# chrismile/LineVis

Measured on AMD Instinct MI355X. Metric: Mrays/s, higher is better.
Workload: dtype f32

## Files before the change

include/linevis_hip.h:

```cpp
#ifndef LINEVIS_HIP_H
#define LINEVIS_HIP_H

#include <stdint.h>

#ifdef __cplusplus
extern "C" {
#endif

#define LV_OK 0
#define LV_E_INVALID (-1)
#define LV_E_HIP (-2)
#define LV_E_STATE (-3)
#define LV_E_CAPACITY (-4)

#define LV_RENDERING_MODE_PER_PIXEL_LINKED_LIST 2
#define LV_RENDERING_MODE_MLAB 3
#define LV_RENDERING_MODE_MBOIT 6
#define LV_RENDERING_MODE_VULKAN_RAY_TRACER 11

typedef struct lv_line_point {
    float linePosition[3];
    float lineAttribute;
    float lineTangent[3];
    float lineRotation;
// ... 5 lines not shown
    float vertexPosition[3];
    uint32_t vertexLinePointIndex;
    float vertexNormal[3];
    float phi;
} lv_tube_vertex;

typedef struct lv_stats {
    uint64_t rays_traced;
    uint64_t nodes_visited;
    uint64_t prims_tested;
    uint64_t hits_shaded;
    uint64_t fragments;
    uint64_t ao_hit_pixels;
    uint32_t max_depth_complexity;
    uint32_t bvh_depth;
    uint32_t num_segments;
    uint32_t num_nodes;
    float ms_accel_build;
    float ms_depth_range;
    float ms_ao;
    float ms_color;
    float ms_ppll_clear;
    float ms_ppll_gather;
    float ms_ppll_resolve;
    float ms_total;
    uint64_t device_bytes;
    float ms_kernel_avg[8];
    uint32_t kernel_launches[8];
    uint64_t ao_rays_traced;
    uint64_t ao_nodes_visited;
    uint64_t ao_prims_tested;
    uint64_t ao_phase_iterations[3];
    uint64_t ao_phase_lanes[3];
    uint32_t max_nodes_per_pixel;
    uint32_t num_tube_triangles;
    uint64_t ppll_pool_nodes;
    uint64_t ao_prim_hits;
    uint64_t ao_prim_may_axis;
    uint64_t ao_prim_may_both;
    float ms_tri_accel_build;
    float ms_tessellate;
    float ms_line_points;
    uint32_t num_tri_nodes;
    uint32_t tri_leaf_bytes;
    uint32_t mboit_degenerate_pixels;
} lv_stats;

#define LV_KERNEL_AO_PRIMARY 0
#define LV_KERNEL_AO_RAYS 1
#define LV_KERNEL_RENDER_RT 2
#define LV_KERNEL_PPLL_GATHER 3
#define LV_KERNEL_PPLL_RESOLVE 4
#define LV_KERNEL_DEPTH_RANGE 5
#define LV_KERNEL_PPLL_SHADE 6
#define LV_KERNEL_PPLL_RASTER 7

typedef struct lv_ctx lv_ctx;

lv_ctx* lv_create(int device_ordinal, int* err);
void lv_destroy(lv_ctx* ctx);
const char* lv_last_error(const lv_ctx* ctx);
const char* lv_version(void);

int lv_set_stream(lv_ctx* ctx, void* hip_stream);

int lv_set_lines(lv_ctx* ctx, const lv_line_point* points, uint32_t num_points,
// ... 116 lines not shown
```

linevis_amd/capi.py:

```python
import ctypes as C
import os

import numpy as np

_HERE = os.path.dirname(os.path.abspath(__file__))
LIB_PATH = os.environ.get("LV_LIB_PATH") or os.path.join(_HERE, "_lib", "liblinevis_hip.so")
HEADER_PATH = os.path.join(os.path.dirname(_HERE), "include", "linevis_hip.h")

LV_OK = 0
MODE_PPLL = 2
MODE_MLAB = 3
MODE_MBOIT = 6
MODE_RAY_TRACER = 11

LINE_POINT_DTYPE = np.dtype([("linePosition", "<f4", 3), ("lineAttribute", "<f4"),
                             ("lineTangent", "<f4", 3), ("lineRotation", "<f4"),
                             ("lineNormal", "<f4", 3), ("lineStartIndex", "<u4")])
assert LINE_POINT_DTYPE.itemsize == 48
TUBE_VERTEX_DTYPE = np.dtype([("vertexPosition", "<f4", 3), ("vertexLinePointIndex", "<u4"),
                              ("vertexNormal", "<f4", 3), ("phi", "<f4")])
assert TUBE_VERTEX_DTYPE.itemsize == 32


class Stats(C.Structure):
    _fields_ = [("rays_traced", C.c_uint64), ("nodes_visited", C.c_uint64), ("prims_tested", C.c_uint64),
                ("hits_shaded", C.c_uint64), ("fragments", C.c_uint64), ("ao_hit_pixels", C.c_uint64),
                ("max_depth_complexity", C.c_uint32), ("bvh_depth", C.c_uint32), ("num_segments", C.c_uint32),
                ("num_nodes", C.c_uint32),
                ("ms_accel_build", C.c_float), ("ms_depth_range", C.c_float), ("ms_ao", C.c_float),
                ("ms_color", C.c_float), ("ms_ppll_clear", C.c_float), ("ms_ppll_gather", C.c_float),
                ("ms_ppll_resolve", C.c_float), ("ms_total", C.c_float), ("device_bytes", C.c_uint64),
                ("ms_kernel_avg", C.c_float * 8), ("kernel_launches", C.c_uint32 * 8),
                ("ao_rays_traced", C.c_uint64), ("ao_nodes_visited", C.c_uint64), ("ao_prims_tested", C.c_uint64),
                ("ao_phase_iterations", C.c_uint64 * 3), ("ao_phase_lanes", C.c_uint64 * 3),
                ("max_nodes_per_pixel", C.c_uint32), ("num_tube_triangles", C.c_uint32),
                ("ppll_pool_nodes", C.c_uint64), ("ao_prim_hits", C.c_uint64), ("ao_prim_may_axis", C.c_uint64),
                ("ao_prim_may_both", C.c_uint64),
                ("ms_tri_accel_build", C.c_float), ("ms_tessellate", C.c_float), ("ms_line_points", C.c_float),
                ("num_tri_nodes", C.c_uint32), ("tri_leaf_bytes", C.c_uint32), ("mboit_degenerate_pixels", C.c_uint32)]

    def as_dict(self):
        d = {}
        for n, _ in self._fields_:
            v = getattr(self, n)
            d[n] = list(v) if hasattr(v, "__len__") else v
        return d


class StreamlineSettings(C.Structure):
    _fields_ = [("integration_method", C.c_uint32), ("integration_direction", C.c_uint32),
                ("time_step_scale", C.c_float), ("max_num_iterations", C.c_int32),
                ("termination_distance", C.c_float), ("minimum_length", C.c_float)]


class HelicitySeedingSettings(C.Structure):
    _fields_ = [("minimum_separation_distance", C.c_float), ("termination_check_type", C.c_uint32), ("loop_check_mode", C.c_uint32),
                ("termination_distance_self", C.c_float), ("seeding_subsampling_factor", C.c_int32)]

    def __init__(self, minimum_separation_distance=0.08, termination_check_type=1, loop_check_mode=1, termination_distance_self=1.0,
                 seeding_subsampling_factor=1):
        super().__init__(minimum_separation_distance, termination_check_type, loop_check_mode, termination_distance_self,
                         seeding_subsampling_factor)


INTEGRATION_METHODS = {"Explicit Euler": 0, "Implicit Euler": 1, "Heun": 2, "Midpoint": 3, "Runge-Kutta 4th Order": 4,
                       "Runge-Kutta-Fehlberg": 5}
INTEGRATION_DIRECTIONS = {"Forward": 0, "Backward": 1, "Forward & Backward": 2}
# ... 489 lines not shown
```

linevis_amd/csrc/lv_api.hip:

```cpp
#include <algorithm>
#include <cmath>
#include <cstdlib>
#include <cstring>

#include "lv_internal.h"

int lv_fail(lv_ctx* ctx, int code, const char* fmt, ...) {
    char buf[1024];
    va_list ap;
    va_start(ap, fmt);
    vsnprintf(buf, sizeof(buf), fmt, ap);
    va_end(ap);
    if (ctx) ctx->lastError = buf;
    return code;
}

int lv_buf_reserve(lv_ctx* ctx, LvDeviceBuffer& b, size_t bytes) {
    if (bytes == 0) bytes = 16;
    if (b.ptr && b.bytes >= bytes) return LV_OK;
    if (b.ptr) {
        LV_HIP(ctx, hipStreamSynchronize(ctx->stream));
        (void)hipFree(b.ptr);
        b.ptr = nullptr;
        b.bytes = 0;
// ... 876 lines not shown
    if (ctx->evFrameValid) {
        s.ms_total = s.ms_depth_range = s.ms_ao = 0.0f;
        s.ms_color = s.ms_ppll_clear = s.ms_ppll_gather = s.ms_ppll_resolve = 0.0f;
        if (ctx->evPhaseRecorded) {
            s.ms_total = ms(2, 3);
            s.ms_depth_range = ms(2, 5);
            s.ms_ao = ms(5, 7);
            if (ctx->lastMode == LV_RENDERING_MODE_VULKAN_RAY_TRACER) s.ms_color = ms(7, 3);
            else { s.ms_ppll_clear = ms(7, 11); s.ms_ppll_gather = ms(11, 13); s.ms_ppll_resolve = ms(13, 3); }
        }
        LvDevCountersHost hc;
        memset(&hc, 0, sizeof(hc));
        if (ctx->counters.ptr) {
            LV_HIP(ctx, hipMemcpy(&hc, ctx->counters.ptr, sizeof(hc), hipMemcpyDeviceToHost));
        }
        s.rays_traced = hc.rays;
        s.nodes_visited = hc.nodes;
        s.prims_tested = hc.prims;
        s.hits_shaded = hc.hits;
        s.fragments = hc.fragCounter;
        s.ao_hit_pixels = hc.aoCount;
        s.max_depth_complexity = hc.maxDepthComplexity;
        s.ao_rays_traced = hc.aoRays;
        s.ao_nodes_visited = hc.aoNodes;
        s.ao_prims_tested = hc.aoPrims;
        s.max_nodes_per_pixel = hc.maxNodesPerPixel;
        s.ao_prim_hits = hc.aoPrimHits;
        s.ao_prim_may_axis = hc.aoPrimMayAxis;
        s.ao_prim_may_both = hc.aoPrimMayBoth;
        s.mboit_degenerate_pixels = hc.mboitDegenerate;
        if (ctx->mboitStreamLast && hc.mboitOverflow)
            return lv_fail(ctx, LV_E_CAPACITY, "MBOIT (streamed): a pixel of the last frame is covered by more than 131071 kept fragments");
        for (int k = 0; k < 3; k++) { s.ao_phase_iterations[k] = hc.aoPhaseIters[k]; s.ao_phase_lanes[k] = hc.aoPhaseLanes[k]; }
    }
    for (int k = 0; k < 8; k++) { s.ms_kernel_avg[k] = 0.0f; s.kernel_launches[k] = 0; }
    for (int k = 0; k < lv_ctx::kNumKernels; k++) {
        const uint64_t n = ctx->kernelLaunches[k];
        const uint64_t m = n < uint64_t(lv_ctx::kRing) ? n : uint64_t(lv_ctx::kRing);
        double sum = 0.0;
        for (uint64_t i = 0; i < m; i++) {
            const uint64_t slot = (n - 1 - i) % lv_ctx::kRing;
            float t = 0.0f;
            if (hipEventElapsedTime(&t, ctx->evKernel[k][2 * slot], ctx->evKernel[k][2 * slot + 1]) == hipSuccess) sum += t;
        }
        s.ms_kernel_avg[k] = m ? float(sum / double(m)) : 0.0f;
        s.kernel_launches[k] = uint32_t(n);
    }
    uint64_t bytes = 0;
    for (const LvDeviceBuffer* b : lv_all_buffers(ctx)) bytes += b->bytes;
    s.device_bytes = bytes;
    *out = s;
    for (int r = 1; aggregate && r < lv_multi_num_ranks(ctx); r++) {
        lv_stats ps;
        const int rc = lv_get_stats_impl(lv_multi_rank(ctx, r), &ps, false);
        if (rc) return lv_fail(ctx, rc, "rank %d: %s", r, lv_multi_rank(ctx, r)->lastError.c_str());
        out->rays_traced += ps.rays_traced; out->nodes_visited += ps.nodes_visited; out->prims_tested += ps.prims_tested;
        out->hits_shaded += ps.hits_shaded; out->fragments += ps.fragments; out->ao_hit_pixels += ps.ao_hit_pixels;
        out->ao_rays_traced += ps.ao_rays_traced; out->ao_nodes_visited += ps.ao_nodes_visited; out->ao_prims_tested += ps.ao_prims_tested;
        out->ao_prim_hits += ps.ao_prim_hits; out->ao_prim_may_axis += ps.ao_prim_may_axis; out->ao_prim_may_both += ps.ao_prim_may_both;
        out->max_depth_complexity = ps.max_depth_complexity > out->max_depth_complexity ? ps.max_depth_complexity : out->max_depth_complexity;
        out->mboit_degenerate_pixels += ps.mboit_degenerate_pixels;
        out->device_bytes += ps.device_bytes;
    }
    (void)hipSetDevice(ctx->device);
    return LV_OK;
}
// ... 380 lines not shown
```

linevis_amd/csrc/lv_device.h:

```cpp
#pragma once

#include <hip/hip_runtime.h>
#include <stdint.h>

#include "../../include/linevis_hip.h"

#define LV_WAVE 64
#define LV_BLOCK 256
#define LV_LEAF_BIT 0x80000000u
#define LV_INVALID 0xFFFFFFFFu
#ifndef LV_STACK_LDS
#define LV_STACK_LDS 24
#endif
#define LV_STACK_SPILL 64
#ifndef LV_RT_MIN_WAVES
#define LV_RT_MIN_WAVES 4
#endif
#ifndef LV_GATHER_MIN_WAVES
#define LV_GATHER_MIN_WAVES 1
#endif
#ifndef LV_PRISM_MIN_WAVES
#define LV_PRISM_MIN_WAVES 3
#endif
#define LV_PPLL_DEAD 0xFFFFFFFFu
// ... 42 lines not shown
#endif
#ifndef LV_NODE_MIN_ACTIVE
#define LV_NODE_MIN_ACTIVE 24
#endif

#ifndef LV_HANDOVER_MAX_BUSY
#define LV_HANDOVER_MAX_BUSY 32
#endif
#ifndef LV_HANDOVER_MAX_BUSY_ALL
#define LV_HANDOVER_MAX_BUSY_ALL 48
#endif
#ifndef LV_HANDOVER_MAX_BUSY_DYN
#define LV_HANDOVER_MAX_BUSY_DYN 24
#endif

#ifndef LV_RESOLVE_LDS_MAX
#define LV_RESOLVE_LDS_MAX (64 * 1024)
#endif
#ifndef LV_RESOLVE_SLAB_GRID
#define LV_RESOLVE_SLAB_GRID 4096u
#endif
#ifndef LV_PPLL_CHUNK
#define LV_PPLL_CHUNK 256
#endif
#ifndef LV_PPLL_SLICES
#define LV_PPLL_SLICES 1
#endif

struct LvDevCounters {
    unsigned long long rays, nodes, prims, hits;
    unsigned long long aoRays, aoNodes, aoPrims;
    unsigned long long aoQueueHead;
    unsigned long long aoPhaseIters[3], aoPhaseLanes[3];
    uint32_t fragCounter;
    uint32_t aoCount;
    uint32_t maxDepthComplexity;
    uint32_t depthOrd[2];
    uint32_t maxNodesPerPixel;
    uint32_t fragAlloc;
    uint32_t prismDiscards;
    uint32_t mlatTraceCount;
    uint32_t ppllOverflowPixels;
    uint32_t prismListCount;
    unsigned long long aoPrimHits, aoPrimMayAxis, aoPrimMayBoth;
    uint32_t mlabLongPixels;
    uint32_t mlabSaturated;
    uint32_t mboitDegenerate;
    uint32_t mboitBoxOrd[6];
    uint32_t mboitOverflow;
};

struct f3 { float x, y, z; };
struct f4 { float x, y, z, w; };

__device__ __forceinline__ f3 mk3(float x, float y, float z) { f3 r; r.x = x; r.y = y; r.z = z; return r; }
__device__ __forceinline__ f3 operator+(f3 a, f3 b) { return mk3(a.x + b.x, a.y + b.y, a.z + b.z); }
__device__ __forceinline__ f3 operator-(f3 a, f3 b) { return mk3(a.x - b.x, a.y - b.y, a.z - b.z); }
__device__ __forceinline__ f3 operator*(f3 a, float s) { return mk3(a.x * s, a.y * s, a.z * s); }
__device__ __forceinline__ f3 operator*(float s, f3 a) { return mk3(s * a.x, s * a.y, s * a.z); }
__device__ __forceinline__ float dot3(f3 a, f3 b) { return (a.x * b.x + a.y * b.y) + a.z * b.z; }
__device__ __forceinline__ f3 cross3(f3 a, f3 b) {
    return mk3(a.y * b.z - b.y * a.z, a.z * b.x - b.z * a.x, a.x * b.y - b.x * a.y);
}
__device__ __forceinline__ float len3(f3 a) { return sqrtf(dot3(a, a)); }
__device__ __forceinline__ f3 norm3(f3 a) { float l = len3(a); return mk3(a.x / l, a.y / l, a.z / l); }
__device__ __forceinline__ float clampf(float x, float lo, float hi) { return fminf(fmaxf(x, lo), hi); }
// ... 260 lines not shown
```

linevis_amd/csrc/lv_render.hip:

```cpp
#include <algorithm>
#include <cmath>
#include <cstring>

#include "lv_internal.h"
#include "lv_trace.h"
#include "lv_tile.h"
#include "lv_mboit.h"

namespace {

#define LV_PRE_HITS 4u
template <bool STATS, int PRIM, int BANDS = LV_SHADE_PLAIN, bool PRE = false, int FAST = 0>
__global__ __launch_bounds__(LV_BLOCK, (STATS || PRIM == LV_PRIM_ELLIPTIC) ? 1 : LV_RT_MIN_WAVES) void k_render_rt(const LvUniforms U, const LvSceneDev S, const LvTiles T,
                                                        uint32_t* __restrict__ out, LvDevCounters* dc,
                                                        const uint2* __restrict__ firstHit = nullptr, const size_t firstHitStride = 0) {
    __shared__ unsigned s_stack[LV_STACK_LDS * LV_BLOCK];
    LV_COOP_SHARED(LV_BLOCK / LV_WAVE);
    LV_COOP_MEM(cm);
    LvPixel px;
    if (!lv_block_pixel(U, T, px)) return;
    const unsigned long long tg0 = lv_group_clock();
    const LvStackMem sm = lv_stack_mem(s_stack, S.stackOverflow);
    LvCounters cnt = {0, 0, 0, 0};
    const bool capped = U.useCappedTubes != 0 || U.lssGeometry != 0;
// ... 306 lines not shown

__global__ __launch_bounds__(LV_BLOCK) void k_ao_tile_scan(const uint32_t* __restrict__ tileCount, uint32_t numTiles,
                                                           uint32_t* __restrict__ tileBase, LvDevCounters* dc) {
    __shared__ uint32_t s_part[LV_BLOCK];
    const uint32_t per = (numTiles + LV_BLOCK - 1u) / LV_BLOCK;
    const uint32_t b = threadIdx.x * per, e = min(b + per, numTiles);
    uint32_t sum = 0;
    for (uint32_t i = b; i < e; i++) sum += tileCount[i];
    s_part[threadIdx.x] = sum;
    __syncthreads();
    if (threadIdx.x == 0) {
        uint32_t run = 0;
        for (uint32_t i = 0; i < LV_BLOCK; i++) { const uint32_t v = s_part[i]; s_part[i] = run; run += v; }
        tileBase[numTiles] = run;
        dc->aoCount = run;
        dc->aoQueueHead = 0ull;
    }
    __syncthreads();
    uint32_t run = s_part[threadIdx.x];
    for (uint32_t i = b; i < e; i++) { tileBase[i] = run; run += tileCount[i]; }
}

__device__ __forceinline__ size_t lv_ao_slot(const uint32_t* __restrict__ tileBase, uint32_t numTiles, const LvAoLayout& tileCapacity,
                                             uint32_t ordinal) {
    if (!tileBase) return ordinal;
    uint32_t lo = 0, hi = numTiles;
    while (hi - lo > 1u) {
        const uint32_t mid = (lo + hi) >> 1;
        if (tileBase[mid] <= ordinal) lo = mid; else hi = mid;
    }
    return lv_ao_group_base(tileCapacity, lo) + (ordinal - tileBase[lo]);
}

#ifndef LV_AO_KEY64
#define LV_AO_KEY64 0
#endif
#if LV_AO_KEY64
typedef unsigned long long lv_ao_key;
__device__ __forceinline__ lv_ao_key lv_ao_key_none(float aoRadius) { return ((unsigned long long)__float_as_uint(aoRadius) << 32) | 0xFFFFFFFFull; }
__device__ __forceinline__ lv_ao_key lv_ao_key_hit(float t, unsigned low) { return ((unsigned long long)__float_as_uint(t) << 32) | low; }
__device__ __forceinline__ float lv_ao_key_t(lv_ao_key key) { return __uint_as_float(unsigned(key >> 32)); }
#else
typedef unsigned lv_ao_key;
__device__ __forceinline__ lv_ao_key lv_ao_key_none(float aoRadius) { return __float_as_uint(aoRadius) + 1u; }
__device__ __forceinline__ lv_ao_key lv_ao_key_hit(float t, unsigned) { return __float_as_uint(t); }
__device__ __forceinline__ float lv_ao_key_t(lv_ao_key key) { return __uint_as_float(key); }
#endif

template <bool BAKE>
__device__ __forceinline__ void lv_ao_generate_ray(const LvUniforms& U, float4 g0, float4 g1, float4 g2, uint32_t smpIdx, uint32_t spp,
                                                   const uint2* __restrict__ lcgSkip, float2* gen) {
    const uint32_t pix = __float_as_uint(g1.w);
    const f3 pos = mk3(g0.x, g0.y, g0.z), T = mk3(g1.x, g1.y, g1.z), N = mk3(g2.x, g2.y, g2.z);
    const f3 B = cross3(N, T);
    uint32_t seed;
    if (BAKE) {
        const uint32_t sub = __float_as_uint(g2.w);
        const uint2 skip = lcgSkip[2u * (sub * spp + smpIdx)];
        seed = skip.x * lv_tea(pix , U.aoFrameNumber) + skip.y;
    } else {
        seed = lv_tea(pix, U.aoGlobalFrameNumber * spp + smpIdx);
    }
    const float xi0 = lv_rnd(seed), xi1 = lv_rnd(seed);
    float sn, cs;
    lv_sincos2pi(xi1, sn, cs);
    const float rs = sqrtf(1.0f - xi0 * xi0);
    const f3 smp = mk3(cs * rs, sn * rs, xi0);
    const f3 dirU = mk3((T.x * smp.x + B.x * smp.y) + N.x * smp.z, (T.y * smp.x + B.y * smp.y) + N.y * smp.z,
                        (T.z * smp.x + B.z * smp.y) + N.z * smp.z);
    const f3 d = norm3(dirU);
    const f3 o = BAKE ? pos : pos + d * g0.w;
    gen[0] = make_float2(o.x, o.y);
    gen[1] = make_float2(o.z, d.x);
    gen[2] = make_float2(d.y, d.z);
}

template <bool STATS, bool ANY_HIT, int PRIM, bool BAKE = false, bool LIT = false, bool PIXEL_GEN = false>
__global__ __launch_bounds__(LV_AO_BLOCK, LV_AO_MIN_WAVES) void k_ao_rays(const LvUniforms U, const LvSceneDev S,
                                                         const float4* __restrict__ gbuf, float* __restrict__ samples,
                                                         LvDevCounters* dc, const uint32_t* __restrict__ tileBase,
                                                         uint32_t numTiles, const LvAoLayout tileCapacity,
                                                         const uint2* __restrict__ lcgSkip = nullptr) {
    __shared__ unsigned s_stack[LV_AO_STACK_LDS * LV_AO_BLOCK];
    __shared__ float2 s_ray[3 * LV_AO_BLOCK];
    __shared__ float2 s_gen[3 * LV_AO_BLOCK];
    __shared__ unsigned s_queue[LV_AO_BLOCK / LV_WAVE][LV_AO_QCAP];
    __shared__ lv_ao_key s_key[LV_AO_BLOCK];
    __shared__ uint4 s_genState[PIXEL_GEN ? LV_AO_BLOCK / LV_WAVE : 1];

    const uint32_t spp = U.aoSamplesPerFrame;
    const unsigned long long total = (unsigned long long)(dc->aoCount) * spp;
    const unsigned chunk = total < (unsigned long long)gridDim.x * (LV_AO_BLOCK / LV_WAVE) * LV_AO_CHUNK * LV_AO_SMALL_CHUNKS ? LV_AO_CHUNK_SMALL
                                                                                                                             : LV_AO_CHUNK;
    const bool capped = U.useCappedTubes != 0;
    const float radius = U.radius;
    const unsigned lane = threadIdx.x & 63u, w = threadIdx.x >> 6;
    const unsigned long long below = (1ull << lane) - 1ull;
    float2* rayW = &s_ray[3 * LV_WAVE * w];
    float2* genW = &s_gen[3 * LV_WAVE * w];
    unsigned* queueW = s_queue[w];
    lv_ao_key* keyW = &s_key[LV_WAVE * w];
    uint4* genStateW = &s_genState[PIXEL_GEN ? w : 0];
    if (PIXEL_GEN && lane == 0) genStateW[0] = make_uint4(0u, 0u, 0u, 0u);
    const lv_ao_key keyInit = lv_ao_key_none(U.aoRadius);
    const float litSlack = PRIM == LV_PRIM_ELLIPTIC ? S.ellBandWidth * 1.001f : (PRIM == LV_PRIM_CAPSULE && LIT) ? radius * 1.001f : 0.0f;

    LvStackT<LV_AO_STACK_LDS, LV_AO_BLOCK> st;
    st.init(&s_stack[threadIdx.x], S.stackOverflow ? S.stackOverflow + (size_t(blockIdx.x) * LV_AO_BLOCK + threadIdx.x) : nullptr,
            gridDim.x * LV_AO_BLOCK);
    LvCounters cnt = {0, 0, 0, 0};
    unsigned long long phIt[3] = {0, 0, 0}, phLn[3] = {0, 0, 0};
    unsigned long long mayAxis = 0, mayBoth = 0, primHits = 0;

    unsigned long long chunkNext = 0, chunkEnd = 0, genBase = 0;
    unsigned genCount = 0, genPos = 0;
    unsigned head = 0, tail = 0;
    bool sourceDry = (S.numSegs == 0) || (total == 0);
    bool hasRay = false, enq = false;
    unsigned long long r = 0;
    f3 inv = mk3(0, 0, 0), oi = mk3(0, 0, 0);
    float best = 0.0f;
    unsigned cur = LV_INVALID, lastSeq = 0;
    unsigned owner = lane;
    constexpr unsigned TB = PRIM == LV_PRIM_TRIANGLE ? LV_AO_TEST_BATCH_TRI : LV_AO_TEST_BATCH;

    while (true) {
        {
            const bool isLeaf = tail - head < LV_WAVE && cur != LV_INVALID && (cur & LV_LEAF_BIT);
            const unsigned long long mL = __ballot(isLeaf);
            if (mL) {
                if (isLeaf) {
                    const unsigned idx = tail + unsigned(__popcll(mL & below));
                    queueW[idx % LV_AO_QCAP] = (owner << 26) | (cur & 0x03FFFFFFu);
                    lastSeq = idx;
                    enq = true;
                    cur = lv_pop_or_done(st);
                }
                tail += unsigned(__popcll(mL));
                if (tail - head < TB) continue;
            }
        }
        const bool canRefill = (genPos < genCount) || !sourceDry;
        const bool drain = !canRefill;
        if (!drain && hasRay && cur == LV_INVALID && (!enq || int(head - lastSeq) > 0)) {
            const lv_ao_key key = keyW[lane];
            float occ = 1.0f;
            if (key != keyInit) occ = U.aoUseDistance ? lv_ao_key_t(key) / U.aoRadius : 0.0f;
            samples[r] = occ;
            hasRay = false;
        }
        const unsigned long long mNode = __ballot(cur != LV_INVALID && !(cur & LV_LEAF_BIT));
        const unsigned long long mIdle = __ballot(!hasRay);
        const int nNode = __popcll(mNode), nIdle = __popcll(mIdle);
        const unsigned q = tail - head;

        if (q >= TB || (q > 0 && nNode == 0 && !(canRefill && nIdle > 0))) {
            const unsigned n = q < LV_WAVE ? q : LV_WAVE;
            __builtin_amdgcn_fence(__ATOMIC_ACQ_REL, "wavefront");
            if (STATS && lane == 0) { phIt[2]++; phLn[2] += n; }
            if (lane < n) {
                const unsigned e = queueW[(head + lane) % LV_AO_QCAP];
                const unsigned owner = e >> 26, leaf = e & 0x03FFFFFFu;
                const float2 r0 = rayW[3 * owner], r1 = rayW[3 * owner + 1], r2 = rayW[3 * owner + 2];
                if (STATS) cnt.prims += PRIM == LV_PRIM_TRIANGLE ? S.triLeafSize : 1u;
                float t; unsigned low;
                if (lv_leaf_test<PRIM, LIT ? 1 : 0>(S, leaf, mk3(r0.x, r0.y, r1.x), mk3(r1.y, r2.x, r2.y), radius, capped, t, low, 0.0f,
                                                    U.aoRadius)) {
                    if (t >= 0.0f && t <= U.aoRadius) {
                        atomicMin(&keyW[owner], lv_ao_key_hit(t, low));
                        if (STATS) primHits++;
                    }
                }
                if (STATS && PRIM == LV_PRIM_CAPSULE) {
                    const float4 sa = S.segs[2 * size_t(leaf)], sb = S.segs[2 * size_t(leaf) + 1];
                    const f3 ro = mk3(r0.x, r0.y, r1.x), rd = mk3(r1.y, r2.x, r2.y);
                    const bool ma = lv_capsule_may_hit_axis(ro, rd, mk3(sa.x, sa.y, sa.z), mk3(sb.x, sb.y, sb.z), radius);
                    const bool mb = lv_capsule_may_hit_sphere(ro, rd, mk3(sa.x, sa.y, sa.z), mk3(sb.x, sb.y, sb.z), radius);
                    mayAxis += ma ? 1u : 0u;
                    mayBoth += (ma && mb) ? 1u : 0u;
                }
            }
            head += n;
            __builtin_amdgcn_fence(__ATOMIC_ACQ_REL, "wavefront");
            {
                const lv_ao_key key = keyW[owner];
                best = lv_ao_key_t(key);
                if (ANY_HIT && key != keyInit) { cur = LV_INVALID; st.sp = 0; }
            }
            continue;
        }
        if (drain) {
            if (nNode == 0) {
                if (hasRay) {
                    const lv_ao_key key = keyW[lane];
                    float occ = 1.0f;
                    if (key != keyInit) occ = U.aoUseDistance ? lv_ao_key_t(key) / U.aoRadius : 0.0f;
                    samples[r] = occ;
                }
                break;
            }
            if (nNode <= LV_HANDOVER_MAX_BUSY) {
                const bool idle = cur == LV_INVALID;
                const bool donor = !idle && st.sp > 0;
                const unsigned long long mFree = __ballot(idle), mDonor = __ballot(donor);
                const unsigned nPairs = min(unsigned(__popcll(mFree)), unsigned(__popcll(mDonor)));
                if (nPairs) {
                    if (donor) {
                        const unsigned rk = unsigned(__popcll(mDonor & below));
                        if (rk < nPairs) genW[rk] = make_float2(__uint_as_float(st.pop()), __uint_as_float(owner));
                    }
                    __builtin_amdgcn_fence(__ATOMIC_ACQ_REL, "wavefront");
                    if (idle) {
                        const unsigned rk = unsigned(__popcll(mFree & below));
                        if (rk < nPairs) {
                            const float2 x = genW[rk];
                            cur = __float_as_uint(x.x);
                            owner = __float_as_uint(x.y);
                            const float2 r0 = rayW[3 * owner], r1 = rayW[3 * owner + 1], r2 = rayW[3 * owner + 2];
                            inv = lv_traversal_inv(mk3(r1.y, r2.x, r2.y));
                            oi = mk3(r0.x * inv.x, r0.y * inv.y, r1.x * inv.z);
                            best = lv_ao_key_t(keyW[owner]);
                            st.sp = 0;
                        }
                    }
                    __builtin_amdgcn_fence(__ATOMIC_ACQ_REL, "wavefront");
                    continue;
                }
            }
        }
        if (canRefill && nIdle > 0 && (nIdle >= LV_REFILL_THRESHOLD || nNode < LV_NODE_MIN_ACTIVE)) {
            if (genPos >= genCount) {
                if (chunkNext >= chunkEnd) {
                    unsigned long long base = 0;
                    if (lane == 0) base = atomicAdd(&dc->aoQueueHead, (unsigned long long)chunk);
                    chunkNext = __shfl(base, 0, 64);
                    chunkEnd = chunkNext + chunk;
                    if (chunkEnd > total) chunkEnd = total;
                    if (chunkNext >= total) { chunkNext = chunkEnd = total; sourceDry = true; }
                }
                const unsigned long long left = chunkEnd - chunkNext;
                const unsigned n = left < LV_WAVE ? unsigned(left) : LV_WAVE;
                if (STATS && lane == 0 && n) { phIt[0]++; phLn[0] += n; }
                if (PIXEL_GEN) {
                    if (n) {
                        const uint32_t b = __builtin_amdgcn_readfirstlane(uint32_t(chunkNext / LV_WAVE)), bpp = spp / LV_WAVE;
                        const uint32_t genOrdinal = bpp == 1u ? b : __builtin_amdgcn_readfirstlane(b / bpp);
                        const uint32_t genSmp0 = (b - genOrdinal * bpp) * LV_WAVE;
                        const uint4 gs = genStateW[0];
                        uint32_t genLo = __builtin_amdgcn_readfirstlane(gs.x), genHi = __builtin_amdgcn_readfirstlane(gs.y);
                        uint32_t genSlot0 = __builtin_amdgcn_readfirstlane(gs.z);
                        if (genOrdinal - genLo >= genHi - genLo) {
                            uint32_t lo = 0, hi = numTiles;
                            while (hi - lo > 1u) {
                                const uint32_t mid = (lo + hi) >> 1;
                                if (tileBase[mid] <= genOrdinal) lo = mid; else hi = mid;
// ... 7 lines not shown
                        const float4 g0 = gbuf[3 * slot + 0], g1 = gbuf[3 * slot + 1], g2 = gbuf[3 * slot + 2];
                        lv_ao_generate_ray<false>(U, g0, g1, g2, genSmp0 + lane, spp, lcgSkip, &genW[3 * lane]);
                    }
                } else if (lane < n) {
                    const unsigned long long rr = chunkNext + lane;
                    const uint32_t smpIdx = uint32_t(rr % spp);
                    const size_t slot = lv_ao_slot(tileBase, numTiles, tileCapacity, uint32_t(rr / spp));
                    const float4 g0 = gbuf[3 * slot + 0], g1 = gbuf[3 * slot + 1], g2 = gbuf[3 * slot + 2];
                    lv_ao_generate_ray<BAKE>(U, g0, g1, g2, smpIdx, spp, lcgSkip, &genW[3 * lane]);
                }
                genBase = chunkNext;
                chunkNext += n;
                genCount = n;
                genPos = 0;
                __builtin_amdgcn_fence(__ATOMIC_ACQ_REL, "wavefront");
            }
            const unsigned avail = genCount - genPos;
            const unsigned k = unsigned(nIdle) < avail ? unsigned(nIdle) : avail;
            if (!hasRay) {
                const unsigned rank = unsigned(__popcll(mIdle & below));
                if (rank < k) {
                    const unsigned gs = genPos + rank;
                    const float2 r0 = genW[3 * gs], r1 = genW[3 * gs + 1], r2 = genW[3 * gs + 2];
                    rayW[3 * lane] = r0;
                    rayW[3 * lane + 1] = r1;
                    rayW[3 * lane + 2] = r2;
                    keyW[lane] = keyInit;
                    inv = lv_traversal_inv(mk3(r1.y, r2.x, r2.y));
                    oi = mk3(r0.x * inv.x, r0.y * inv.y, r1.x * inv.z);
                    best = U.aoRadius;
                    r = genBase + gs;
                    owner = lane;
                    cur = 0;
                    st.sp = 0;
                    enq = false;
                    hasRay = true;
                    if (STATS) cnt.rays++;
                }
            }
            genPos += k;
            __builtin_amdgcn_fence(__ATOMIC_ACQ_REL, "wavefront");
            continue;
        }
        if (nNode > 0) {
            int nNow;
            do {
                if (STATS && lane == 0) { phIt[1]++; }
                if (STATS && !(cur & LV_LEAF_BIT)) phLn[1]++;
                if (!(cur & LV_LEAF_BIT)) cur = lv_node_step<STATS>(S, cur, oi, inv, 0.0f - litSlack, best + litSlack, st, cnt);
                const bool isLeaf = cur != LV_INVALID && (cur & LV_LEAF_BIT);
                const unsigned long long mL = __ballot(isLeaf);
                if (mL) {
                    if (isLeaf) {
                        const unsigned idx = tail + unsigned(__popcll(mL & below));
                        queueW[idx % LV_AO_QCAP] = (owner << 26) | (cur & 0x03FFFFFFu);
                        lastSeq = idx;
                        enq = true;
                        cur = lv_pop_or_done(st);
                    }
                    tail += unsigned(__popcll(mL));
                }
                nNow = __popcll(__ballot(!(cur & LV_LEAF_BIT)));
            } while (tail - head < TB && nNow >= (drain ? LV_HANDOVER_MAX_BUSY + 1 : 1));
            continue;
        }
        if (nIdle == LV_WAVE && !canRefill) break;
    }
    if (STATS) {
        lv_flush_counters(cnt, dc, true);
        for (int k = 0; k < 3; k++) {
            const unsigned long long it = lv_wave_sum_u64(phIt[k]), ln = lv_wave_sum_u64(phLn[k]);
            if (lane == 0) { atomicAdd(&dc->aoPhaseIters[k], it); atomicAdd(&dc->aoPhaseLanes[k], ln); }
        }
        const unsigned long long sa = lv_wave_sum_u64(mayAxis), sb = lv_wave_sum_u64(mayBoth), sh = lv_wave_sum_u64(primHits);
        if (lane == 0) { atomicAdd(&dc->aoPrimMayAxis, sa); atomicAdd(&dc->aoPrimMayBoth, sb); atomicAdd(&dc->aoPrimHits, sh); }
    }
}

template <bool BAKE>
__global__ __launch_bounds__(LV_BLOCK) void k_ao_reduce(const LvUniforms U, const float4* __restrict__ gbuf,
                                                        const float* __restrict__ samples, const float* aoIn, float* ao,
                                                        const LvDevCounters* dc, const uint32_t* __restrict__ tileBase,
                                                        uint32_t numTiles, const LvAoLayout tileCapacity) {
    const uint32_t slot = blockIdx.x * LV_BLOCK + threadIdx.x;
    if (slot >= dc->aoCount) return;
    const uint32_t spp = U.aoSamplesPerFrame;
    float aoFactor = 0.0f;
    if ((spp & 3u) == 0u) {
        const float4* row = reinterpret_cast<const float4*>(samples + size_t(slot) * spp);
        for (uint32_t s = 0; s < spp / 4u; s++) {
            const float4 v = row[s];
            aoFactor += v.x; aoFactor += v.y; aoFactor += v.z; aoFactor += v.w;
        }
    } else {
        for (uint32_t s = 0; s < spp; s++) aoFactor += samples[size_t(slot) * spp + s];
    }
    aoFactor /= float(spp);
    const uint32_t pix = BAKE ? slot : __float_as_uint(gbuf[3 * lv_ao_slot(tileBase, numTiles, tileCapacity, slot) + 1].w);
    if (U.aoFrameNumber != 0) aoFactor = mixf(aoIn[pix], aoFactor, 1.0f / float(U.aoFrameNumber + 1));
    ao[pix] = aoFactor;
}

#define LV_REDUCE_ROWS 128u
__global__ __launch_bounds__(LV_REDUCE_ROWS) void k_ao_reduce_rows(const LvUniforms U, const float4* __restrict__ gbuf,
                                                                   const float* __restrict__ samples, const float* aoIn, float* ao,
                                                                   const LvDevCounters* dc, const uint32_t* __restrict__ tileBase,
                                                                   uint32_t numTiles, const LvAoLayout tileCapacity) {
// ... 3418 lines not shown
```

linevis_amd/csrc/lv_trace.h:

```cpp
#pragma once

#include "lv_device.h"

__device__ __forceinline__ bool lv_ray_sphere(f3 o, f3 d, f3 ctr, float radius, float& hitT) {
    f3 f = o - ctr;
    float A = dot3(d, d);
    float tc = -dot3(f, d) / A;
    f3 l = f + tc * d;
    float disc = radius * radius - dot3(l, l);
    if (disc < 0.0f) return false;
    float h = sqrtf(disc / A);
    float t0 = tc - h;
    float t1 = tc + h;
    hitT = t0;
    if (t0 >= 0.0f) hitT = t0;
    else if (t1 >= 0.0f) hitT = t1;
    else return false;
    return true;
}

__device__ __forceinline__ bool lv_ray_tube_td(f3 o, f3 d, f3 tubeStart, f3 tubeEnd, f3 td, float radius, float& hitT) {
    f3 deltaP = o - tubeStart;
    f3 av = d - dot3(d, td) * td;
    f3 cv = deltaP - dot3(deltaP, td) * td;
// ... 119 lines not shown
    const f3 m = cross3(w, d);
    const float d2 = dot3(d, d), w2 = dot3(w, w);
    const float R = (0.5f * __builtin_sqrtf(dot3(v, v)) + radius) * 1.0001f;
    return dot3(m, m) <= R * R * d2 + 1e-5f * (w2 * d2) * R + 1e-30f;
}

__device__ __forceinline__ bool lv_ray_triangle(f3 o, f3 d, f3 inv, f3 v0, f3 v1, f3 v2, float pad, float& tOut, float& uOut,
                                                float& vOut) {
    const f3 e1 = v1 - v0, e2 = v2 - v0;
    const f3 p = cross3(d, e2);
    const float det = dot3(e1, p);
    if (det == 0.0f) return false;
    const float r = 1.0f / det;
    const f3 tv = o - v0;
    const float u = dot3(tv, p) * r;
    if (!(u >= 0.0f && u <= 1.0f)) return false;
    const f3 q = cross3(tv, e1);
    const float v = dot3(d, q) * r;
    if (!(v >= 0.0f && u + v <= 1.0f)) return false;
    const float t = dot3(e2, q) * r;
    const float mnx = fminf(fminf(v0.x, v1.x), v2.x) - pad, mxx = fmaxf(fmaxf(v0.x, v1.x), v2.x) + pad;
    const float mny = fminf(fminf(v0.y, v1.y), v2.y) - pad, mxy = fmaxf(fmaxf(v0.y, v1.y), v2.y) + pad;
    const float mnz = fminf(fminf(v0.z, v1.z), v2.z) - pad, mxz = fmaxf(fmaxf(v0.z, v1.z), v2.z) + pad;
    const float tx0 = (mnx - o.x) * inv.x, tx1 = (mxx - o.x) * inv.x;
    const float ty0 = (mny - o.y) * inv.y, ty1 = (mxy - o.y) * inv.y;
    const float tz0 = (mnz - o.z) * inv.z, tz1 = (mxz - o.z) * inv.z;
    const float tn = fmaxf(fmaxf(fminf(tx0, tx1), fminf(ty0, ty1)), fminf(tz0, tz1));
    const float tf = fminf(fminf(fmaxf(tx0, tx1), fmaxf(ty0, ty1)), fmaxf(tz0, tz1));
    if (!(t >= tn && t <= tf)) return false;
    tOut = t; uOut = u; vOut = v;
    return true;
}

typedef __attribute__((address_space(3))) unsigned lv_lds_u32;
typedef __attribute__((address_space(1))) unsigned lv_glb_u32;

template <int NLDS, int STRIDE = LV_BLOCK>
struct LvStackT {
    static constexpr int kLds = NLDS;
    static constexpr int kStride = STRIDE;
    lv_lds_u32* lds;
    lv_glb_u32* ovf;
    unsigned ovfStride;
    int sp;
    __device__ __forceinline__ void init(unsigned* ldsBase, unsigned* ovfBase, unsigned stride) {
        lds = (lv_lds_u32*)ldsBase; ovf = (lv_glb_u32*)ovfBase; ovfStride = stride; sp = 0;
    }
    __device__ __forceinline__ void push(unsigned v) {
        if (sp < NLDS) lds[sp * STRIDE] = v;
        else ovf[size_t(sp - NLDS) * ovfStride] = v;
        sp++;
    }
    __device__ __forceinline__ unsigned pop() {
        sp--;
        unsigned v;
        if (sp < NLDS) v = lds[sp * STRIDE];
        else v = ovf[size_t(sp - NLDS) * ovfStride];
        return v;
    }
};
typedef LvStackT<LV_STACK_LDS> LvStack;
struct LvStackMem {
    unsigned* lds;
    unsigned* ovf;
    unsigned ovfStride;
};
__device__ __forceinline__ LvStackMem lv_stack_mem(unsigned* sStack, unsigned* ovfSlab) {
    LvStackMem m;
    m.lds = sStack + threadIdx.x;
    m.ovfStride = gridDim.x * LV_BLOCK;
    m.ovf = ovfSlab ? ovfSlab + (size_t(blockIdx.x) * LV_BLOCK + threadIdx.x) : nullptr;
    return m;
}

struct LvHit {
    float t;
    uint32_t leaf;
    int kind;
    bool found;
};

template <class STACK>
__device__ __forceinline__ unsigned lv_pop_or_done(STACK& st) { return st.sp == 0 ? LV_INVALID : st.pop(); }

__device__ __forceinline__ void lv_cswap(float& ka, unsigned& ca, float& kb, unsigned& cb) {
    const bool sw = kb < ka;
    const float tk = sw ? kb : ka, uk = sw ? ka : kb;
    const unsigned tc = sw ? cb : ca, uc = sw ? ca : cb;
    ka = tk; kb = uk; ca = tc; cb = uc;
}

__device__ __forceinline__ bool lv_slab_q(uint32_t nearX, uint32_t nearY, uint32_t nearZ, uint32_t farX, uint32_t farY,
                                          uint32_t farZ, int k, f3 A, f3 B, float tMin, float tMax, float& tNear) {
    const float tx0 = __builtin_fmaf(float((nearX >> (8 * k)) & 0xFFu), A.x, B.x);
    const float ty0 = __builtin_fmaf(float((nearY >> (8 * k)) & 0xFFu), A.y, B.y);
    const float tz0 = __builtin_fmaf(float((nearZ >> (8 * k)) & 0xFFu), A.z, B.z);
    const float tx1 = __builtin_fmaf(float((farX >> (8 * k)) & 0xFFu), A.x, B.x);
    const float ty1 = __builtin_fmaf(float((farY >> (8 * k)) & 0xFFu), A.y, B.y);
    const float tz1 = __builtin_fmaf(float((farZ >> (8 * k)) & 0xFFu), A.z, B.z);
    const float tn = fmaxf(fmaxf(tx0, ty0), fmaxf(tz0, tMin));
    const float tf = fminf(fminf(tx1, ty1), fminf(tz1, tMax));
    tNear = tn;
    return tn <= __builtin_fmaf(tf, 1.00001f, 4e-7f);
}

#ifndef LV_TRAVERSAL_INV_IEEE
#define LV_TRAVERSAL_INV_IEEE 0
#endif
__device__ __forceinline__ f3 lv_traversal_inv(f3 d) {
#if LV_TRAVERSAL_INV_IEEE
    return mk3(1.0f / d.x, 1.0f / d.y, 1.0f / d.z);
#else
    return mk3(__builtin_amdgcn_rcpf(d.x), __builtin_amdgcn_rcpf(d.y), __builtin_amdgcn_rcpf(d.z));
#endif
}

// ... 1367 lines not shown
```

Before: 5331.

## Add sentinel-based AO stack, drop enq flag, and continue traversal after refill

The AO ray kernel's traversal stack gains a sentinel slot holding LV_INVALID, so popping an empty stack needs no branch. The per-lane enq flag is replaced by initialising lastSeq to head-1 when a new ray starts. After a refill pass the wave now falls through to node traversal in the same outer iteration when enough lanes are busy, instead of always looping back. A static_assert keeps LDS under 32 KB to preserve occupancy, and a STATS-only outer-pass counter is added. The trade-off is one extra LDS slot per thread and a changed refill/traversal schedule that could alter how lanes stay converged.

```diff
diff --git a/include/linevis_hip.h b/include/linevis_hip.h
--- a/include/linevis_hip.h
+++ b/include/linevis_hip.h
@@ -61,6 +61,7 @@
     uint64_t ao_prims_tested;
     uint64_t ao_phase_iterations[3];
     uint64_t ao_phase_lanes[3];
+    uint64_t ao_outer_passes;
     uint32_t max_nodes_per_pixel;
     uint32_t num_tube_triangles;
     uint64_t ppll_pool_nodes;
diff --git a/linevis_amd/capi.py b/linevis_amd/capi.py
--- a/linevis_amd/capi.py
+++ b/linevis_amd/capi.py
@@ -32,7 +32,7 @@
                 ("ms_ppll_resolve", C.c_float), ("ms_total", C.c_float), ("device_bytes", C.c_uint64),
                 ("ms_kernel_avg", C.c_float * 8), ("kernel_launches", C.c_uint32 * 8),
                 ("ao_rays_traced", C.c_uint64), ("ao_nodes_visited", C.c_uint64), ("ao_prims_tested", C.c_uint64),
-                ("ao_phase_iterations", C.c_uint64 * 3), ("ao_phase_lanes", C.c_uint64 * 3),
+                ("ao_phase_iterations", C.c_uint64 * 3), ("ao_phase_lanes", C.c_uint64 * 3), ("ao_outer_passes", C.c_uint64),
                 ("max_nodes_per_pixel", C.c_uint32), ("num_tube_triangles", C.c_uint32),
                 ("ppll_pool_nodes", C.c_uint64), ("ao_prim_hits", C.c_uint64), ("ao_prim_may_axis", C.c_uint64),
                 ("ao_prim_may_both", C.c_uint64),
diff --git a/linevis_amd/csrc/lv_api.hip b/linevis_amd/csrc/lv_api.hip
--- a/linevis_amd/csrc/lv_api.hip
+++ b/linevis_amd/csrc/lv_api.hip
@@ -932,6 +932,7 @@
         if (ctx->mboitStreamLast && hc.mboitOverflow)
             return lv_fail(ctx, LV_E_CAPACITY, "MBOIT (streamed): a pixel of the last frame is covered by more than 131071 kept fragments");
         for (int k = 0; k < 3; k++) { s.ao_phase_iterations[k] = hc.aoPhaseIters[k]; s.ao_phase_lanes[k] = hc.aoPhaseLanes[k]; }
+        s.ao_outer_passes = hc.aoOuterPasses;
     }
     for (int k = 0; k < 8; k++) { s.ms_kernel_avg[k] = 0.0f; s.kernel_launches[k] = 0; }
     for (int k = 0; k < lv_ctx::kNumKernels; k++) {
diff --git a/linevis_amd/csrc/lv_device.h b/linevis_amd/csrc/lv_device.h
--- a/linevis_amd/csrc/lv_device.h
+++ b/linevis_amd/csrc/lv_device.h
@@ -98,6 +98,7 @@
     unsigned long long aoRays, aoNodes, aoPrims;
     unsigned long long aoQueueHead;
     unsigned long long aoPhaseIters[3], aoPhaseLanes[3];
+    unsigned long long aoOuterPasses;
     uint32_t fragCounter;
     uint32_t aoCount;
     uint32_t maxDepthComplexity;
diff --git a/linevis_amd/csrc/lv_render.hip b/linevis_amd/csrc/lv_render.hip
--- a/linevis_amd/csrc/lv_render.hip
+++ b/linevis_amd/csrc/lv_render.hip
@@ -362,6 +362,9 @@
     return lv_ao_group_base(tileCapacity, lo) + (ordinal - tileBase[lo]);
 }
 
+#ifndef LV_AO_REFILL_DESCEND
+#define LV_AO_REFILL_DESCEND 1
+#endif
 #ifndef LV_AO_KEY64
 #define LV_AO_KEY64 0
 #endif
@@ -411,12 +414,14 @@
                                                          LvDevCounters* dc, const uint32_t* __restrict__ tileBase,
                                                          uint32_t numTiles, const LvAoLayout tileCapacity,
                                                          const uint2* __restrict__ lcgSkip = nullptr) {
-    __shared__ unsigned s_stack[LV_AO_STACK_LDS * LV_AO_BLOCK];
+    __shared__ unsigned s_stack[(LV_AO_STACK_LDS + LV_AO_STACK_SENTINEL) * LV_AO_BLOCK];
     __shared__ float2 s_ray[3 * LV_AO_BLOCK];
     __shared__ float2 s_gen[3 * LV_AO_BLOCK];
     __shared__ unsigned s_queue[LV_AO_BLOCK / LV_WAVE][LV_AO_QCAP];
     __shared__ lv_ao_key s_key[LV_AO_BLOCK];
     __shared__ uint4 s_genState[PIXEL_GEN ? LV_AO_BLOCK / LV_WAVE : 1];
+    static_assert(sizeof(s_stack) + sizeof(s_ray) + sizeof(s_gen) + sizeof(s_queue) + sizeof(s_key) + sizeof(s_genState) <= 32768,
+                  "k_ao_rays: more than 32 KB of LDS per workgroup costs the fifth workgroup per CU");
 
     const uint32_t spp = U.aoSamplesPerFrame;
     const unsigned long long total = (unsigned long long)(dc->aoCount) * spp;
@@ -435,18 +440,18 @@
     const lv_ao_key keyInit = lv_ao_key_none(U.aoRadius);
     const float litSlack = PRIM == LV_PRIM_ELLIPTIC ? S.ellBandWidth * 1.001f : (PRIM == LV_PRIM_CAPSULE && LIT) ? radius * 1.001f : 0.0f;
 
-    LvStackT<LV_AO_STACK_LDS, LV_AO_BLOCK> st;
+    LvStackT<LV_AO_STACK_LDS + LV_AO_STACK_SENTINEL, LV_AO_BLOCK, true> st;
     st.init(&s_stack[threadIdx.x], S.stackOverflow ? S.stackOverflow + (size_t(blockIdx.x) * LV_AO_BLOCK + threadIdx.x) : nullptr,
             gridDim.x * LV_AO_BLOCK);
     LvCounters cnt = {0, 0, 0, 0};
     unsigned long long phIt[3] = {0, 0, 0}, phLn[3] = {0, 0, 0};
-    unsigned long long mayAxis = 0, mayBoth = 0, primHits = 0;
+    unsigned long long mayAxis = 0, mayBoth = 0, primHits = 0, outerPasses = 0;
 
     unsigned long long chunkNext = 0, chunkEnd = 0, genBase = 0;
     unsigned genCount = 0, genPos = 0;
     unsigned head = 0, tail = 0;
     bool sourceDry = (S.numSegs == 0) || (total == 0);
-    bool hasRay = false, enq = false;
+    bool hasRay = false;
     unsigned long long r = 0;
     f3 inv = mk3(0, 0, 0), oi = mk3(0, 0, 0);
     float best = 0.0f;
@@ -455,6 +460,7 @@
     constexpr unsigned TB = PRIM == LV_PRIM_TRIANGLE ? LV_AO_TEST_BATCH_TRI : LV_AO_TEST_BATCH;
 
     while (true) {
+        if (STATS && lane == 0) outerPasses++;
         {
             const bool isLeaf = tail - head < LV_WAVE && cur != LV_INVALID && (cur & LV_LEAF_BIT);
             const unsigned long long mL = __ballot(isLeaf);
@@ -463,7 +469,6 @@
                     const unsigned idx = tail + unsigned(__popcll(mL & below));
                     queueW[idx % LV_AO_QCAP] = (owner << 26) | (cur & 0x03FFFFFFu);
                     lastSeq = idx;
-                    enq = true;
                     cur = lv_pop_or_done(st);
                 }
                 tail += unsigned(__popcll(mL));
@@ -472,7 +477,7 @@
         }
         const bool canRefill = (genPos < genCount) || !sourceDry;
         const bool drain = !canRefill;
-        if (!drain && hasRay && cur == LV_INVALID && (!enq || int(head - lastSeq) > 0)) {
+        if (!drain && hasRay && cur == LV_INVALID && int(head - lastSeq) > 0) {
             const lv_ao_key key = keyW[lane];
             float occ = 1.0f;
             if (key != keyInit) occ = U.aoUseDistance ? lv_ao_key_t(key) / U.aoRadius : 0.0f;
@@ -481,7 +486,7 @@
         }
         const unsigned long long mNode = __ballot(cur != LV_INVALID && !(cur & LV_LEAF_BIT));
         const unsigned long long mIdle = __ballot(!hasRay);
-        const int nNode = __popcll(mNode), nIdle = __popcll(mIdle);
+        int nNode = __popcll(mNode), nIdle = __popcll(mIdle);
         const unsigned q = tail - head;
 
         if (q >= TB || (q > 0 && nNode == 0 && !(canRefill && nIdle > 0))) {
@@ -515,7 +520,7 @@
             {
                 const lv_ao_key key = keyW[owner];
                 best = lv_ao_key_t(key);
-                if (ANY_HIT && key != keyInit) { cur = LV_INVALID; st.sp = 0; }
+                if (ANY_HIT && key != keyInit) { cur = LV_INVALID; st.reset(); }
             }
             continue;
         }
@@ -531,7 +536,7 @@
             }
             if (nNode <= LV_HANDOVER_MAX_BUSY) {
                 const bool idle = cur == LV_INVALID;
-                const bool donor = !idle && st.sp > 0;
+                const bool donor = !idle && !st.empty();
                 const unsigned long long mFree = __ballot(idle), mDonor = __ballot(donor);
                 const unsigned nPairs = min(unsigned(__popcll(mFree)), unsigned(__popcll(mDonor)));
                 if (nPairs) {
@@ -550,7 +555,7 @@
                             inv = lv_traversal_inv(mk3(r1.y, r2.x, r2.y));
                             oi = mk3(r0.x * inv.x, r0.y * inv.y, r1.x * inv.z);
                             best = lv_ao_key_t(keyW[owner]);
-                            st.sp = 0;
+                            st.reset();
                         }
                     }
                     __builtin_amdgcn_fence(__ATOMIC_ACQ_REL, "wavefront");
@@ -624,15 +629,22 @@
                     r = genBase + gs;
                     owner = lane;
                     cur = 0;
-                    st.sp = 0;
-                    enq = false;
+                    st.reset();
+                    lastSeq = head - 1u;
                     hasRay = true;
                     if (STATS) cnt.rays++;
                 }
             }
             genPos += k;
             __builtin_amdgcn_fence(__ATOMIC_ACQ_REL, "wavefront");
+#if LV_AO_REFILL_DESCEND
+            nNode += int(k);
+            nIdle -= int(k);
+            if (k == 0u || !((genPos < genCount) || !sourceDry) || (nIdle > 0 && (nIdle >= LV_REFILL_THRESHOLD || nNode < LV_NODE_MIN_ACTIVE)))
+                continue;
+#else
             continue;
+#endif
         }
         if (nNode > 0) {
             int nNow;
@@ -647,7 +659,6 @@
                         const unsigned idx = tail + unsigned(__popcll(mL & below));
                         queueW[idx % LV_AO_QCAP] = (owner << 26) | (cur & 0x03FFFFFFu);
                         lastSeq = idx;
-                        enq = true;
                         cur = lv_pop_or_done(st);
                     }
                     tail += unsigned(__popcll(mL));
@@ -665,6 +676,8 @@
             if (lane == 0) { atomicAdd(&dc->aoPhaseIters[k], it); atomicAdd(&dc->aoPhaseLanes[k], ln); }
         }
         const unsigned long long sa = lv_wave_sum_u64(mayAxis), sb = lv_wave_sum_u64(mayBoth), sh = lv_wave_sum_u64(primHits);
+        const unsigned long long so = lv_wave_sum_u64(outerPasses);
+        if (lane == 0) atomicAdd(&dc->aoOuterPasses, so);
         if (lane == 0) { atomicAdd(&dc->aoPrimMayAxis, sa); atomicAdd(&dc->aoPrimMayBoth, sb); atomicAdd(&dc->aoPrimHits, sh); }
     }
 }
diff --git a/linevis_amd/csrc/lv_trace.h b/linevis_amd/csrc/lv_trace.h
--- a/linevis_amd/csrc/lv_trace.h
+++ b/linevis_amd/csrc/lv_trace.h
@@ -175,20 +175,27 @@
     return true;
 }
 
+#ifndef LV_AO_STACK_SENTINEL
+#define LV_AO_STACK_SENTINEL 1
+#endif
 typedef __attribute__((address_space(3))) unsigned lv_lds_u32;
 typedef __attribute__((address_space(1))) unsigned lv_glb_u32;
 
-template <int NLDS, int STRIDE = LV_BLOCK>
+template <int NLDS, int STRIDE = LV_BLOCK, bool AO = false>
 struct LvStackT {
     static constexpr int kLds = NLDS;
     static constexpr int kStride = STRIDE;
+    static constexpr int kEmpty = (AO && LV_AO_STACK_SENTINEL) ? 1 : 0;
     lv_lds_u32* lds;
     lv_glb_u32* ovf;
     unsigned ovfStride;
     int sp;
     __device__ __forceinline__ void init(unsigned* ldsBase, unsigned* ovfBase, unsigned stride) {
-        lds = (lv_lds_u32*)ldsBase; ovf = (lv_glb_u32*)ovfBase; ovfStride = stride; sp = 0;
-    }
+        lds = (lv_lds_u32*)ldsBase; ovf = (lv_glb_u32*)ovfBase; ovfStride = stride; sp = kEmpty;
+        if (kEmpty) lds[0] = LV_INVALID;
+    }
+    __device__ __forceinline__ void reset() { sp = kEmpty; if (kEmpty) lds[0] = LV_INVALID; }
+    __device__ __forceinline__ bool empty() const { return sp <= kEmpty; }
     __device__ __forceinline__ void push(unsigned v) {
         if (sp < NLDS) lds[sp * STRIDE] = v;
         else ovf[size_t(sp - NLDS) * ovfStride] = v;
@@ -224,7 +231,10 @@
 };
 
 template <class STACK>
-__device__ __forceinline__ unsigned lv_pop_or_done(STACK& st) { return st.sp == 0 ? LV_INVALID : st.pop(); }
+__device__ __forceinline__ unsigned lv_pop_or_done(STACK& st) {
+    if (STACK::kEmpty) return st.pop();
+    return st.sp == 0 ? LV_INVALID : st.pop();
+}
 
 __device__ __forceinline__ void lv_cswap(float& ka, unsigned& ca, float& kb, unsigned& cb) {
     const bool sw = kb < ka;
```

After: 5626, median of 6. +5.5%, better.
